# raguilar011095/planet_heightmap_generation

Hardware: AMD Instinct MI355X
Metric: Mcells·iter/s, terrain-post erosion stack (higher is better)
Workload: dtype f64

## Files before the change

### planet_heightmap_generation_amd/csrc/device.h

```cpp
#pragma once
#include <hip/hip_runtime.h>

#include <cstdint>
#include <cstdio>
#include <map>
#include <string>
#include <utility>
#include <vector>

#include "device_mem.h"
#include "host_util.h"

#include "erode_ops.h"
#include "flood_ops.h"
#include "wo_internal.h"

namespace wo {

#define WO_TRY try {
#define WO_CATCH(fn)                                                                                   \
    } catch (const ::wo::HipError& e) { ::wo::set_error(std::string(fn) + ": " + e.msg); return 2; }   \
      catch (const std::exception& e) { ::wo::set_error(std::string(fn) + ": " + e.what()); return 3; }

#define WO_LOCAL __attribute__((visibility("hidden")))
// ... 16 lines not shown
    const int64_t b = (n + WO_BLOCK - 1) / WO_BLOCK, per = 8 * (int64_t)xcd_tile(n);
    return (int)(((b + per - 1) / per) * per);
}

enum Family : int {
    FAM_COAST = 0, FAM_SMOOTH, FAM_SHARPEN, FAM_CREEP, FAM_WARP, FAM_NOISE, FAM_SYNTH, FAM_OCEAN,
    FAM_SORT_KEYS, FAM_SORT_RADIX, FAM_RANK, FAM_RECEIVERS, FAM_FLOW_SNAP, FAM_FLOW_FINAL,
    FAM_SOLVE_SETUP, FAM_SOLVE_ROUND, FAM_SOLVE_FINAL, FAM_THERMAL_EXCESS, FAM_THERMAL_APPLY,
    FAM_GLAC_INDEX, FAM_ICE_RECV, FAM_ICE_ROUND, FAM_CARVE_SETUP, FAM_CARVE_ROUND, FAM_MORAINE, FAM_GLAC_BLEND,
    FAM_SOLVE_PATCH, FAM_ELEV_COLLISION, FAM_ELEV_MAIN, FAM_PLATE_GRID, FAM_PLATE_PROJECT, FAM_SMOOTH_FIELD,
    FAM_FLOOD_EVAL, FAM_FLOOD_APPLY, FAM_FLOOD_MISC, FAM_CLIMATE, FAM_BASIN, FAM_BASIN_SORT, FAM_SOLVE_BASIN, FAM_FLOW_TILES, FAM_MISC, FAM_EVENT_PAIR, FAM_EVENT_PAIR_NOOP, FAM_EVENT_PAIR_NOOP2,
    FAM_MAP_LONLAT, FAM_MAP_FILL, FAM_MAP_SIDES, FAM_MAP_BIG_BOXES, FAM_MAP_RESOLVE, FAM_MAP_REGION_COLORS, FAM_MAP_PIXELS,
    FAM_MAP_RANGE, FAM_MAP_LAYER_COLORS,
    FAM_GLOBE_TABLES, FAM_GLOBE_REGION_COLORS, FAM_GLOBE_RANGE, FAM_GLOBE_MESH, FAM_GLOBE_LINE_COUNT, FAM_GLOBE_LINE_SCAN, FAM_GLOBE_LINE_WRITE,
    FAM_OVERLAY_BINS, FAM_OVERLAY_ARROWS,
    FAM_PICK, FAM_PICK_REDUCE, FAM_HIGHLIGHT, FAM_COUNT
};
extern const char* const kFamilyNames[FAM_COUNT];

}

struct wo_ctx {
    int device = 0;
    hipStream_t stream = nullptr;
    hipDeviceProp_t prop{};
};

struct wo_flood_gpu {
    wo::DeviceArena mem;
    int64_t version = -1; int32_t L = 0, cap = 0, nSeeds = 0;
    int32_t *off = nullptr, *adj = nullptr, *cell = nullptr, *seedIdx = nullptr, *seeds = nullptr; double* nz = nullptr;
    float* e = nullptr;
    wo::FlHead *A = nullptr, *P = nullptr, *F = nullptr;
    unsigned long long *Astk = nullptr, *Pstk = nullptr, *Fstk = nullptr;
    int32_t *fdEpoch = nullptr, *inDirty = nullptr; uint8_t* isPending = nullptr;
    int32_t* lists[5] = {nullptr, nullptr, nullptr, nullptr, nullptr};
    void* ctrl = nullptr; void* h_ctrl = nullptr;
    int32_t *jump = nullptr, *outPar = nullptr, *outRoot = nullptr; float* outSurf = nullptr;
    int32_t *h_par = nullptr, *h_root = nullptr; float* h_surf = nullptr;
};

namespace wo {
struct Options {
    bool layoutIndex = false;
    bool tileLds = false;
    bool floodDevice = false;
    bool floodTiming = false;
    bool stageTimingAll = false;
    int  relaxedSortEvery = 1;
    bool relaxedFull = false;
    bool basinScramble = false;
    long long carveBudgetMs = 200;
    int  carveBlocks = 0;
    bool oceanSplitSmooth = false;
    bool tempSplitDiffuse = false;
    bool globeDirectStores = false;
    bool overlayPrecheck = false;
    int  pickBlocks = 0;
    static Options from_env();
};
}

struct wo_planet {
    wo_ctx* ctx = nullptr;
    wo::Options opt;
    int32_t N = 0, E = 0, maxDeg = 0;
    wo::DeviceArena mem;
    wo::hvec<int32_t> h_off, h_adj;
    wo::hvec<float> h_xyz;
    wo::hvec<uint8_t> h_ocean;
    bool h_ocean_valid = false;
    float* h_pinned = nullptr;
    int32_t* h_count = nullptr;
    float* d_redoE = nullptr; int32_t* d_pendingEver = nullptr; int64_t redoCalls = 0;
    unsigned long long *h_word = nullptr, *d_word = nullptr; uint32_t wordSerial = 0;
    wo::FloodScratch flood;
    wo::FloodExchange floodX;
    void* floodLink = nullptr; void (*floodLinkFree)(void*) = nullptr;
    wo_flood_gpu fgpu;

    int32_t *d_off = nullptr, *d_adj = nullptr;
    float *d_dist = nullptr, *d_xyz = nullptr;
    float *d_e = nullptr, *d_e2 = nullptr, *d_hot = nullptr, *d_orig = nullptr;
    uint8_t *d_ocean = nullptr, *d_coast = nullptr;
    int64_t mirrorMaskVersion = -1;
    uint8_t* d_oceanKnown = nullptr; int32_t* d_maskDiff = nullptr; bool oceanKnownValid = false;
    bool hot_valid = false;
    float* d_savedE = nullptr; uint8_t* d_savedOcean = nullptr; bool saved = false;
    uint8_t* d_tables = nullptr;
    bool scratch = false;
    bool landIdentity = false;
    int64_t floodPrefixMirror = -1, floodPrefixStatic = -1;
    bool floodPrefixOk = false;
    int32_t *d_landIdx = nullptr, *d_land[2] = {nullptr, nullptr}, *d_rank = nullptr;
    int32_t* d_landInit = nullptr; int64_t oceanVersion = 0, landListsOcean = -1; bool landListsMirror = false; int32_t landListsL = -1;
    uint32_t* d_keys[2] = {nullptr, nullptr};
    float *d_cellDist = nullptr, *d_flow = nullptr;
    wo::SolveTask* d_task = nullptr; wo::SolveOut* d_out = nullptr;
    int32_t *d_haloSend = nullptr, *d_haloRecv = nullptr; float *d_haloBuf = nullptr, *h_haloBuf = nullptr; int32_t nHaloSend = 0, nHaloRecv = 0;
    int32_t* d_flowCnt = nullptr; wo::TargetRank* d_tr = nullptr; wo::EventList* d_ev = nullptr; float* d_me = nullptr;
    int32_t *d_carveSlot = nullptr, *d_carveDeps = nullptr, *d_carveDepCnt = nullptr, *d_carveDepPos = nullptr;
    uint32_t* d_rs[2] = {nullptr, nullptr}; int rsFlip[2] = {0, 0};
    wo::CarveRec* d_carveRecs = nullptr; wo::CarveExpect* d_carveExpect = nullptr; unsigned long long* d_carveG = nullptr;
    int32_t* d_carveSlotDone = nullptr; int64_t carveCap = 0;
    unsigned long long* d_accCnt = nullptr;
    int32_t *d_ftLr = nullptr, *d_ftParent = nullptr, *d_ftExtCnt = nullptr; uint32_t* d_ftInflow = nullptr; unsigned long long* d_ftRootAcc = nullptr;
// ... 137 lines not shown
```

### planet_heightmap_generation_amd/csrc/erode.hip

```cpp
#include <hip/hip_runtime.h>

#include <algorithm>
#include <chrono>
#include <cmath>

#include "../../include/worogen.h"
#include "device.h"
#include "flood.h"
#include "kernels_impl.h"
#include "mirror.h"
#include "stage_clock.h"

namespace wo {

__global__ __launch_bounds__(WO_BLOCK) void k_fill_i32(int32_t* a, int32_t v, int32_t n) { WO_GRID_STRIDE(i, n) a[i] = v; }

constexpr int WO_PATCH_TOTAL_SLOTS = 4096;

static void ensure_scratch(wo_planet* p) {
    if (p->scratch) return;
    const size_t N = (size_t)p->N;
    DeviceArena a;
    p->d_landIdx = a.dev<int32_t>(N); p->d_land[0] = a.dev<int32_t>(N); p->d_land[1] = a.dev<int32_t>(N);
    p->d_keys[0] = a.dev<uint32_t>(N); p->d_keys[1] = a.dev<uint32_t>(N);
// ... 27 lines not shown
        return 1;
    }
    int32_t* tot = p->d_patchTotals;
    int64_t launches = 0;
    constexpr int spinCap = WO_PATCH_SPIN_CAP, lateFrom = WO_PATCH_LATE_FROM, lateCap = WO_PATCH_LATE_SPIN_CAP;
    int64_t need = 0;
    for (int32_t tag = 1;; ) {
        const int32_t first = tag;
        const int burst = (tag == 1) ? std::max<int>(1, (int)std::min<int64_t>(p->lastPatchLaunches, WO_PATCH_TOTAL_SLOTS / 2)) : 3;
        for (int b = 0; b < burst; ++b, ++tag) {
            if (tag % WO_PATCH_TOTAL_SLOTS == 0) {
                if (b > 0) break;
                WO_HIP(hipMemsetAsync(tot, 0, (size_t)WO_PATCH_TOTAL_SLOTS * sizeof(int32_t), s));
            }
            if (tag == 1) basin_solve_launch(p, F, tag, tot + 1);
            else {
                if (tag == 2 && F.solveLean) launch(p, FAM_MISC, k_solve_blk_init, blocks_for(p->L, 4096), WO_BLOCK, F, p->L);
                launch(p, FAM_SOLVE_PATCH, k_solve_patch, np, WO_PATCH_THREADS, F, p->L, tag, p->d_patchPending, tot + (tag % WO_PATCH_TOTAL_SLOTS), K, m, dt,
                       (int32_t*)nullptr, (int32_t)(tag >= lateFrom ? lateCap : spinCap));
            }
            ++launches;
        }
        if (first == 1 && tag == 2) {
            if (read_count(p, tot + 1) == 0) need = 1;
        } else {
            WO_HIP(hipMemcpyAsync(p->h_patchTotals, tot, (size_t)WO_PATCH_TOTAL_SLOTS * sizeof(int32_t), hipMemcpyDeviceToHost, s));
            WO_HIP(hipStreamSynchronize(s));
            for (int32_t t = first; t < tag && !need; ++t) if (p->h_patchTotals[t % WO_PATCH_TOTAL_SLOTS] == 0) need = t;
        }
        if (need) break;
        if (launches > 4 * (int64_t)p->N + 1024) throw HipError{"patch solve does not converge"};
    }
    p->lastPatchLaunches = need;
    return need;
}

static void ensure_side_stream(wo_planet* p) {
    if (p->side) return;
    int prLeast = 0, prGreatest = 0;
    WO_HIP(hipDeviceGetStreamPriorityRange(&prLeast, &prGreatest));
    WO_HIP(hipStreamCreateWithPriority(&p->side, hipStreamNonBlocking, prGreatest));
    WO_HIP(hipEventCreateWithFlags(&p->evFork, hipEventDisableTiming)); WO_HIP(hipEventCreateWithFlags(&p->evJoin, hipEventDisableTiming));
}

struct RedoWithChecks {};

struct ErodeCall {
    wo_planet* p;
    int32_t hIters; double K, m, dt; int32_t tIters; double talus, kThermal; int32_t gIters; double gStrength; bool checkEveryPass;
    int32_t total, midIter; double gCarve, gConv, gDep, gFjord;
    int gridN, gridL = 0;
    StageClock clk; MirrorScope mir; FloodRun floodRun;
    int64_t sorts = 0, maxSolve = 0, patchLaunches = 0, basinPasses = 0, basinLeftoverPasses = 0, iceRounds = 0, carveRounds = 0, carveActive = 0, carveFlowLeft = 0;
    double floodHostMs = 0;
    ErodeCall(wo_planet* pl, int32_t h, double K_, double m_, double dt_, int32_t t, double talus_, double kT, int32_t g, double gs, bool check)
        : p(pl), hIters(h), K(K_), m(m_), dt(dt_), tIters(t), talus(talus_), kThermal(kT), gIters(std::max(g, 0)), gStrength(gs != gs ? 0 : gs),
          checkEveryPass(check), total(std::max(hIters, std::max(tIters, gIters))), midIter((int32_t)std::floor(total * 0.75 + 0.5)),
          gridN(xcd_grid(pl->N)), clk(pl), mir(pl) {
        const double gScale = gIters > 0 ? 1.0 / gIters : 0;
        gCarve = 0.02 * gScale; gConv = 0.01 * gScale; gDep = 0.005 * gScale; gFjord = 0.015 * gScale;
    }
    void stats(bool mirrored) const {
        p->erodeStats = {{"land_cells", (double)p->L}, {"mirror_layout", mirrored ? 1.0 : 0.0}, {"iterations", (double)total}, {"sorts", (double)sorts},
                         {"solve_launches_max_per_pass", (double)maxSolve}, {"solve_patch_launches_total", (double)patchLaunches},
                         {"solve_basin_passes", (double)basinPasses}, {"solve_basin_passes_with_leftovers", (double)basinLeftoverPasses},
                         {"flow_two_level", (p->d_ftLr && p->landIdentity && hIters > 0) ? 1.0 : 0.0}, {"ice_rounds_total", (double)iceRounds},
                         {"carve_rounds_total", (double)carveRounds}, {"carve_active_total", (double)carveActive}, {"carve_flow_launches_with_leftovers", (double)carveFlowLeft}, {"solve_check_every_pass", checkEveryPass ? 1.0 : 0.0}, {"calls_run_again_with_checks", (double)p->redoCalls}, {"flood_stage_ms", floodHostMs},
                         {"flood_device_pass1_ms", floodRun.deviceMs}, {"flood_device_rounds", (double)floodRun.rounds}, {"flood_device_epochs", (double)floodRun.epochs},
                         {"flood_device_evaluations", (double)floodRun.evals}, {"flood_equal_key_decisions", (double)floodRun.ties}, {"flood_pass1_on_host", (floodRun.usedDevice && !floodRun.fellBack) ? 0.0 : 1.0},
                         {"flood_host_calls", (double)floodRun.host.calls}, {"flood_host_serial_pass1", (double)floodRun.host.serialPass1}, {"flood_host_tie_groups", (double)floodRun.host.tieGroups}, {"flood_host_contested", (double)floodRun.host.contested},
                         {"flood_host_open_parents", (double)floodRun.host.openParents}, {"flood_host_unresolved", (double)floodRun.host.unresolved},
                         {"flood_host_path_redo", (double)floodRun.host.pathRedo}, {"flood_host_replays", (double)floodRun.host.replays}, {"flood_host_replayed_landmasses", (double)floodRun.host.replayedLandmasses}, {"flood_host_pass1_ms", floodRun.host.pass1Ms},
                         {"flood_host_pass23_ms", floodRun.host.pass23Ms},
                         {"relaxed_sort_every", (double)p->opt.relaxedSortEvery}, {"relaxed_full", p->opt.relaxedFull ? 1.0 : 0.0}, {"flood_exchange_calls", (double)p->floodX.calls}, {"flood_exchange_gathers", (double)p->floodX.gathers}, {"flood_exchange_whole_planet_floods", (double)p->floodX.globalFloods}, {"flood_exchange_received", (double)p->floodX.received}};
    }
};
template <class Cell>
static int32_t compact_land(int64_t n, const uint8_t* ocean, Cell cell, int32_t* out) {
    std::vector<int64_t> cnt(host_threads() + 2, 0);
    parallel_ranges(n, [&](int64_t b, int64_t e, int t) { int64_t c = 0; for (int64_t i = b; i < e; ++i) c += ocean[cell(i)] ? 0 : 1; cnt[t + 1] = c; });
    for (size_t t = 1; t < cnt.size(); ++t) cnt[t] += cnt[t - 1];
    parallel_ranges(n, [&](int64_t b, int64_t e, int t) { int64_t o = cnt[t]; for (int64_t i = b; i < e; ++i) if (!ocean[cell(i)]) out[o++] = (int32_t)i; });
    return (int32_t)cnt.back();
}
static void erode_without_land(ErodeCall& c) {
    wo_planet* p = c.p;
    if (p->floodX.on) {
        hipStream_t s = p->ctx->stream;
        const int calls = (c.hIters > 0 ? 1 : 0) + (c.midIter < c.total ? 1 : 0);
        WO_HIP(hipMemcpyAsync(p->h_pinned, c.mir.on ? p->mirror.o_e : p->d_e, (size_t)p->N * sizeof(float), hipMemcpyDeviceToHost, s));
        WO_HIP(hipStreamSynchronize(s));
        ensure_flood_static(p);
        for (int k = 0; k < calls; ++k) flood_exchange(p, 0.5, nullptr);
    }
    c.mir.finish();
    c.clk.end(); c.clk.finish();
}
static bool erode_setup(ErodeCall& c) {
    wo_planet* p = c.p; hipStream_t s = p->ctx->stream;
    const int32_t N = p->N;
    c.clk.begin("setup");
    refresh_host_ocean(p);
    c.mir.enter(p->h_ocean.data());
    p->landIdentity = c.mir.on && p->mirror.h_mask.size() == (size_t)N;
    coast_flags(p);
    int32_t* hl = reinterpret_cast<int32_t*>(p->h_pinned);
    const uint8_t* oc = p->h_ocean.data();
    const bool listsKept = p->d_landInit && p->landListsOcean == p->oceanVersion && p->landListsMirror == c.mir.on && p->landListsL >= 0;
    const int32_t L = listsKept ? p->landListsL : compact_land(N, oc, [](int64_t r) { return r; }, hl);
    p->L = L;
    if (L == 0) { erode_without_land(c); return false; }
    if (listsKept) {
        WO_HIP(hipMemcpyAsync(p->d_land[0], p->d_landInit, (size_t)L * sizeof(int32_t), hipMemcpyDeviceToDevice, s));
    } else if (c.mir.on) {
        WO_HIP(hipMemcpyAsync(p->d_listA, hl, (size_t)L * sizeof(int32_t), hipMemcpyHostToDevice, s));
        mirror_map_i32(p, p->d_listA, p->d_land[0], L);
        WO_HIP(hipStreamSynchronize(s));
        const int32_t* perm = p->mirror.h_perm.data();
        compact_land(N, oc, [perm](int64_t i) { return perm[i]; }, hl);
        WO_HIP(hipMemcpyAsync(p->d_landIdx, hl, (size_t)L * sizeof(int32_t), hipMemcpyHostToDevice, s));
    } else {
        WO_HIP(hipMemcpyAsync(p->d_landIdx, hl, (size_t)L * sizeof(int32_t), hipMemcpyHostToDevice, s));
        WO_HIP(hipMemcpyAsync(p->d_land[0], p->d_landIdx, (size_t)L * sizeof(int32_t), hipMemcpyDeviceToDevice, s));
    }
    if (!listsKept) {
        if (!p->d_landInit) p->d_landInit = p->mem.dev<int32_t>((size_t)N);
        WO_HIP(hipMemcpyAsync(p->d_landInit, p->d_land[0], (size_t)L * sizeof(int32_t), hipMemcpyDeviceToDevice, s));
        p->landListsOcean = p->oceanVersion; p->landListsMirror = c.mir.on; p->landListsL = L;
    }
    WO_HIP(hipStreamSynchronize(s));
    p->landCur = 0;
    launch(p, FAM_MISC, k_init_rank, c.gridN, WO_BLOCK, p->d_rank, N);
    rank_from_land(p);
    if (c.hIters > 0) {
        ensure_flood_static(p);
        if (p->patchVersion != p->flood.staticVersion || p->patchMirror != c.mir.on) {
            p->patchMirror = c.mir.on;
            if (c.mir.on) WO_HIP(hipMemcpyAsync(p->d_patchOrder, p->d_landIdx, (size_t)L * sizeof(int32_t), hipMemcpyDeviceToDevice, s));
            else WO_HIP(hipMemcpyAsync(p->d_patchOrder, p->flood.landCell.data(), (size_t)L * sizeof(int32_t), hipMemcpyHostToDevice, s));
            launch(p, FAM_MISC, k_fill_i32, c.gridN, WO_BLOCK, p->d_slotOf, -1, N);
            launch(p, FAM_MISC, k_slot_scatter, blocks_for(L, 4096), WO_BLOCK, (const int32_t*)p->d_patchOrder, p->d_slotOf, L);
            WO_HIP(hipStreamSynchronize(s));
            p->patchVersion = p->flood.staticVersion;
            p->lastPatchLaunches = 1;
            p->numPatches = (L + WO_PATCH - 1) / WO_PATCH;
        }
    } else p->patchVersion = -1;
    c.gridL = xcd_grid(L);
    if (c.hIters > 0 || c.tIters > 0) {
        WO_HIP(hipMemcpyAsync(p->d_e2, p->d_e, (size_t)N * sizeof(float), hipMemcpyDeviceToDevice, s));
        launch(p, FAM_MISC, k_erode_ocean_init, blocks_for(N, 4096), WO_BLOCK, p->fields());
    }
    c.clk.end();
    return true;
}
static void leftovers_so_far(ErodeCall& c) {
    wo_planet* p = c.p;
    if (c.checkEveryPass || !p->d_pendingEver || read_count(p, p->d_pendingEver) == 0) return;
    if (p->opt.floodTiming) {
        int32_t h[8] = {0};
        WO_HIP(hipMemcpy(h, p->d_pendingEver, sizeof(h), hipMemcpyDeviceToHost));
        std::fprintf(stderr, "[erode] call runs again with checks: %d basin-solve tasks were left pending\n", h[0]);
    }
    throw RedoWithChecks{};
}
static void erode_flood(ErodeCall& c, double carveStrength) {
    wo_planet* p = c.p;
    leftovers_so_far(c);
    c.clk.begin("priority_flood");
    const auto t0 = std::chrono::steady_clock::now();
    const bool landOnly = c.mir.on && p->landIdentity && !p->floodX.on && !p->opt.floodDevice && p->h_ocean_valid && p->flood.staticValid &&
                          p->flood.staticN == p->N && p->flood.L > 0 && flood_land_is_mirror_prefix(p);
    if (landOnly) flood_stage_land(p, carveStrength, c.floodRun);
    else { c.mir.suspend(); flood_stage(p, carveStrength, c.floodRun); c.mir.resume(); }
    c.floodHostMs += std::chrono::duration<double, std::milli>(std::chrono::steady_clock::now() - t0).count();
    c.clk.end();
}
static void erode_sort(ErodeCall& c) { c.clk.begin("sort"); sort_land_by_elevation(c.p); ++c.sorts; c.clk.end(); }
static void ice_flow(ErodeCall& c, const Fields& F) {
    launch(c.p, FAM_ICE_RECV, k_ice_receivers, c.gridN, WO_BLOCK, F);
    launch(c.p, FAM_ICE_ROUND, k_ice_climb, c.gridL, WO_BLOCK, F, F.blocker); ++c.iceRounds;
}
static void glacial_step_relaxed(ErodeCall& c) {
    wo_planet* p = c.p;
    c.clk.begin("glacial");
    const Fields F = p->fields();
    ice_flow(c, F);
    launch(p, FAM_CARVE_ROUND, k_carve_jacobi, c.gridL, WO_BLOCK, F, (const float*)p->d_e, p->d_e2, c.gCarve, c.gConv, c.gStrength);
    swap_elev(p);
    launch(p, FAM_MORAINE, k_moraine_fjord, c.gridN, WO_BLOCK, p->fields(), c.gDep, c.gFjord);
    c.clk.end();
}
static void ensure_carve_capacity(wo_planet* p, int32_t active) {
    if ((int64_t)active <= p->carveCap) return;
    DeviceArena& a = p->mem;
    a.release(p->d_carveDeps); a.release(p->d_carveDepCnt); a.release(p->d_carveDepPos); a.release(p->d_carveRecs); a.release(p->d_carveSlotDone); a.release(p->d_carveExpect);
    p->carveCap = 0;
    const size_t cap = (size_t)active + active / 4 + 1024;
    p->d_carveDeps = a.dev<int32_t>(cap * WO_CARVE_DEPS);
    p->d_carveDepCnt = a.dev<int32_t>(cap); p->d_carveDepPos = a.dev<int32_t>(cap);
    p->d_carveRecs = a.dev<CarveRec>(cap); p->d_carveSlotDone = a.dev<int32_t>(cap); p->d_carveExpect = a.dev<CarveExpect>(cap);
    p->carveCap = (int64_t)cap;
}
static int carve_granule_blocks() {
    static int blocks = 0;
    if (!blocks) {
        int perCu = 0, dev = 0; hipDeviceProp_t prop;
        WO_HIP(hipOccupancyMaxActiveBlocksPerMultiprocessor(&perCu, k_carve_granules, WO_BLOCK, 0));
        WO_HIP(hipGetDevice(&dev)); WO_HIP(hipGetDeviceProperties(&prop, dev));
        blocks = std::max(1, std::min(perCu, 8) - 1) * prop.multiProcessorCount;
    }
    return blocks;
}
static int64_t carve_launches(ErodeCall& c, const Fields& F, int32_t active) {
    wo_planet* p = c.p;
    const int32_t* const count = p->d_counters + 3; int32_t* const done = p->d_counters + 4;
    launch(p, FAM_CARVE_SETUP, k_carve_records, blocks_for(active), WO_BLOCK, F, (const int32_t*)p->d_listB, count, p->d_carveRecs, p->d_carveSlotDone, c.gCarve, c.gConv, c.gStrength,
           (int32_t)0, (int32_t)1);
    WO_HIP(hipMemsetAsync(done, 0, sizeof(int32_t), p->ctx->stream));
    const int grid = blocks_for(active);
    const int blocksNow = p->opt.carveBlocks > 0 ? std::max(1, std::min(carve_granule_blocks(), p->opt.carveBlocks)) : carve_granule_blocks();
    const long long flowBudget = p->opt.carveBudgetMs * 100000ll;
    if (!p->d_carveG) p->d_carveG = p->mem.dev<unsigned long long>((size_t)p->N);
    launch(p, FAM_CARVE_SETUP, k_carve_expect, grid, WO_BLOCK, F, (const CarveRec*)p->d_carveRecs, count, p->d_carveExpect);
    launch(p, FAM_CARVE_SETUP, k_carve_pack, blocks_for(p->N, 4096), WO_BLOCK, (const float*)F.e, p->d_carveG, p->N);
    launch(p, FAM_CARVE_ROUND, k_carve_granules, std::min(grid, blocksNow), WO_BLOCK, F, (const CarveRec*)p->d_carveRecs, (const CarveExpect*)p->d_carveExpect, p->d_carveG,
           p->d_carveSlotDone, count, done, flowBudget);
    launch(p, FAM_CARVE_SETUP, k_carve_unpack, blocks_for(p->N, 4096), WO_BLOCK, (const unsigned long long*)p->d_carveG, F.e, p->N);
    int64_t k = 2;
    if (read_count(p, done) >= active) return k - 1;
    ++c.carveFlowLeft;
    launch(p, FAM_CARVE_SETUP, k_carve_deps, grid, WO_BLOCK, F, (const int32_t*)p->d_listB, count, p->d_carveSlot);
    launch(p, FAM_CARVE_SETUP, k_carve_records, grid, WO_BLOCK, F, (const int32_t*)p->d_listB, count, p->d_carveRecs, p->d_carveSlotDone, c.gCarve, c.gConv, c.gStrength, (int32_t)1, (int32_t)0);
    constexpr int burst = 32;
    for (;;) {
        for (int b = 0; b < burst; ++b, ++k)
            launch(p, FAM_CARVE_ROUND, k_carve_round_static, grid, WO_BLOCK, F, (const CarveRec*)p->d_carveRecs, p->d_carveSlotDone, count, (int32_t)k, c.gCarve, c.gConv, c.gStrength, done);
        if (read_count(p, done) >= active) return k - 1;
        if (k > 4 * (int64_t)p->N + 1024) throw HipError{"carve rounds do not converge"};
    }
}
static void glacial_step_exact(ErodeCall& c) {
    wo_planet* p = c.p;
    c.clk.begin("glacial");
    Fields F = p->fields();
    ice_flow(c, F);
    launch(p, FAM_CARVE_SETUP, k_carve_setup_cells, c.gridN, WO_BLOCK, F);
    select_active_by_rank(p, F.arank, p->d_listB, p->d_counters + 3);
    const int32_t active = read_count(p, p->d_counters + 3);
    c.carveActive += active; ensure_carve_capacity(p, active);
    F.carveDeps = p->d_carveDeps; F.carveDepCnt = p->d_carveDepCnt; F.carveDepPos = p->d_carveDepPos;
    if (active > 0) c.carveRounds += carve_launches(c, F, active);
    launch(p, FAM_MORAINE, k_moraine_fjord, c.gridN, WO_BLOCK, F, c.gDep, c.gFjord);
    c.clk.end();
}
static FlowTiles flow_tiles_buffers(wo_planet* p) {
    const size_t N = (size_t)p->N;
    if (!p->d_ftLr) {
        DeviceArena& a = p->mem;
        if (!p->d_ftParent) p->d_ftParent = a.dev<int32_t>(N);
        if (!p->d_ftExtCnt) p->d_ftExtCnt = a.dev<int32_t>(N);
        if (!p->d_ftInflow) p->d_ftInflow = a.dev<uint32_t>(N);
        if (!p->d_ftRootAcc) p->d_ftRootAcc = a.dev<unsigned long long>(N);
        p->d_ftLr = a.dev<int32_t>(N);
        WO_HIP(hipMemsetAsync(p->d_ftInflow, 0, N * 4, p->ctx->stream)); WO_HIP(hipMemsetAsync(p->d_ftExtCnt, 0, N * 4, p->ctx->stream));
    }
    FlowTiles FT{};
    FT.lr = p->d_ftLr; FT.parent = p->d_ftParent; FT.rootAcc = p->d_ftRootAcc; FT.inflow = p->d_ftInflow; FT.extCnt = p->d_ftExtCnt;
    return FT;
}
static int flow_tile_count(int32_t L) { return (int)(((int64_t)L + FT_CELLS - 1) / FT_CELLS); }
static void erode_receivers(ErodeCall& c, const Fields& F, const FlowTiles& FT, int32_t* donorCnt, bool basin, bool slotIdentity, bool tilesBeforeFork) {
    wo_planet* p = c.p; hipStream_t s = p->ctx->stream;
    Fields Fr = F; if (basin) Fr.basinJ = p->d_basinJ;
    c.clk.begin("receivers");
    launch(p, FAM_RECEIVERS, k_receivers_flow_init, c.gridL, WO_BLOCK, Fr, donorCnt);
    c.clk.end();
    if (!basin) return;
    ensure_side_stream(p);
    if (tilesBeforeFork) {
        launch(p, FAM_FLOW_TILES, k_flow_tiles<false>, flow_tile_count(p->L), FT_THREADS, F, FT);
        launch(p, FAM_FLOW_TILES, k_flow_root_links, blocks_for(p->L, 4096), WO_BLOCK, F, FT);
    }
    WO_HIP(hipEventRecord(p->evFork, s));
    WO_HIP(hipStreamWaitEvent(p->side, p->evFork, 0));
    p->onSide = true;
    try { basin_layout(p, slotIdentity); } catch (...) { p->onSide = false; throw; }
    p->onSide = false;
    WO_HIP(hipEventRecord(p->evJoin, p->side));
}
static void erode_flow(ErodeCall& c, const Fields& F, const FlowTiles& FT, int32_t* donorCnt, bool flowTiles, bool tilesBeforeFork, bool clearOut) {
    wo_planet* p = c.p;
    c.clk.begin("flow");
    if (flowTiles) {
        const int tiles = flow_tile_count(p->L);
        if (!tilesBeforeFork) {
            launch(p, FAM_FLOW_TILES, k_flow_tiles<false>, tiles, FT_THREADS, F, FT);
            launch(p, FAM_FLOW_TILES, k_flow_root_links, blocks_for(p->L, 4096), WO_BLOCK, F, FT);
        }
        launch(p, FAM_FLOW_TILES, k_flow_root_climb, blocks_for(p->L, 4096), WO_BLOCK, F, FT);
        launch(p, FAM_FLOW_TILES, k_flow_tiles<true>, tiles, FT_THREADS, F, FT);
    } else
        launch(p, FAM_FLOW_SNAP, k_flow_climb, c.gridL, WO_BLOCK, F, (const int32_t*)p->d_flowCnt, (int32_t)0x7fffffff);
    Fields Ff = F;
    if (p->opt.relaxedFull) Ff.ev = nullptr;
// ... 41 lines not shown
    erode_flow(c, F, FT, donorCnt, flowTiles, tilesBeforeFork, basin && c.checkEveryPass);
    c.clk.begin("solve");
    if (basin) erode_solve_basin(c, F, iter); else erode_solve_affine(c, F);
    swap_elev(p);
    c.clk.end();
}
static void thermal_step(ErodeCall& c, bool afterSolve) {
    wo_planet* p = c.p;
    c.clk.begin("thermal");
    const Fields F = p->fields();
    if (!afterSolve) launch(p, FAM_THERMAL_EXCESS, k_masked_elev, c.gridL, WO_BLOCK, F);
    launch(p, FAM_THERMAL_EXCESS, k_thermal_excess, c.gridL, WO_BLOCK, F, c.talus);
    if (p->maxDeg <= 12) launch(p, FAM_THERMAL_APPLY, k_thermal_apply_reg<12>, c.gridL, WO_BLOCK, F, p->d_e2, c.talus, c.kThermal);
    else if (p->maxDeg <= 16) launch(p, FAM_THERMAL_APPLY, k_thermal_apply_reg<16>, c.gridL, WO_BLOCK, F, p->d_e2, c.talus, c.kThermal);
    else launch_shmem(p, FAM_THERMAL_APPLY, k_thermal_apply, c.gridL, WO_BLOCK, (size_t)p->maxDeg * WO_BLOCK * 12, F, p->d_e2, c.talus, c.kThermal, (int32_t)p->maxDeg);
    swap_elev(p);
    c.clk.end();
}

static void erode_composite(wo_planet* p, int32_t hIters, double K, double m, double dt, int32_t tIters, double talus,
                            double kThermal, int32_t gIters, double gStrength, bool checkEveryPass = true) {
    ErodeCall c(p, hIters, K, m, dt, tIters, talus, kThermal, gIters, gStrength, checkEveryPass);
    release_stage_brackets(p);
    p->stageTiming.clear(); p->erodeStats.clear();
    p->floodX.calls = 0; p->floodX.gathers = 0; p->floodX.globalFloods = 0; p->floodX.received = 0;
    if (c.total <= 0) return;
    ensure_scratch(p);
    hipStream_t s = p->ctx->stream;
    if (hIters > 0) WO_HIP(hipMemsetAsync(p->d_flowCnt, 0, (size_t)p->N * sizeof(int32_t), s));
    if (hIters > 0 && p->d_ftInflow) { WO_HIP(hipMemsetAsync(p->d_ftInflow, 0, (size_t)p->N * 4, s)); WO_HIP(hipMemsetAsync(p->d_ftExtCnt, 0, (size_t)p->N * 4, s)); }
    if (!erode_setup(c)) return;
    if (hIters > 0) erode_flood(c, 0.5);

    const bool glacial = c.gIters > 0 && c.gStrength > 0;
    if (glacial) launch(p, FAM_GLAC_INDEX, k_glac_index, c.gridN, WO_BLOCK, p->fields(), c.gStrength);
    const bool relaxedFull = p->opt.relaxedFull;
    bool midDone = false, sortAfterFlood = false;
    for (int32_t iter = 0; iter < c.total; ++iter) {
        c.clk.on = true;
        if (!midDone && iter >= c.midIter) { midDone = true; erode_flood(c, 0.85); sortAfterFlood = true; }
        c.clk.on = p->opt.stageTimingAll || p->profiling || c.total <= 16 || iter % 8 == 0;
        const bool gNow = iter < c.gIters && glacial, hNow = iter < hIters;
        const bool sortNow = relaxedFull ? (iter == 0 || sortAfterFlood) : (p->opt.relaxedSortEvery <= 1 || iter % p->opt.relaxedSortEvery == 0);
        if ((gNow || hNow) && sortNow) { sortAfterFlood = false; erode_sort(c); }
        if (gNow) { if (relaxedFull) glacial_step_relaxed(c); else glacial_step_exact(c); }
        if (hNow) {
            if (gNow && sortNow) erode_sort(c);
            hydraulic_step(c, iter);
        }
        if (iter < tIters) thermal_step(c, hNow);
    }
    c.clk.on = true;
    leftovers_so_far(c);
    if (glacial) {
        c.clk.begin("glacial_blend");
        launch(p, FAM_GLAC_BLEND, k_glacial_blend, c.gridN, WO_BLOCK, p->fields(), (const float*)p->d_e, p->d_e2);
        swap_elev(p);
        c.clk.end();
    }
    const bool mirrored = c.mir.on;
    if (mirrored) { c.clk.begin("setup"); c.mir.finish(); c.clk.end(); }
    c.clk.finish();
    c.stats(mirrored);
}

static void erode_composite_checked(wo_planet* p, int32_t hIters, double K, double m, double dt, int32_t tIters, double talus,
                                    double kThermal, int32_t gIters, double gStrength) {
    if (hIters <= 0 || p->floodX.on) { erode_composite(p, hIters, K, m, dt, tIters, talus, kThermal, gIters, gStrength, true); return; }
    hipStream_t s = p->ctx->stream;
    if (!p->d_redoE) p->d_redoE = p->mem.dev<float>((size_t)p->N);
    if (!p->d_pendingEver) p->d_pendingEver = p->mem.dev<int32_t>(16);
    WO_HIP(hipMemcpyAsync(p->d_redoE, p->d_e, (size_t)p->N * sizeof(float), hipMemcpyDeviceToDevice, s));
    WO_HIP(hipMemsetAsync(p->d_pendingEver, 0, 16 * sizeof(int32_t), s));
    try {
        erode_composite(p, hIters, K, m, dt, tIters, talus, kThermal, gIters, gStrength, false);
    } catch (const RedoWithChecks&) {
        WO_HIP(hipStreamSynchronize(s));
        if (p->side) WO_HIP(hipStreamSynchronize(p->side));
        WO_HIP(hipMemcpyAsync(p->d_e, p->d_redoE, (size_t)p->N * sizeof(float), hipMemcpyDeviceToDevice, s));
        ++p->redoCalls;
        erode_composite(p, hIters, K, m, dt, tIters, talus, kThermal, gIters, gStrength, true);
    }
}

}

using namespace wo;

extern "C" {

int wo_erode_composite_resident(wo_planet* p, int32_t hIters, double K, double m, double dt, int32_t tIters, double talusSlope,
                                double kThermal, int32_t gIters, double glacialStrength) {
    if (!check_planet(p, "wo_erode_composite_resident")) return 1;
    WO_TRY
    erode_composite_checked(p, hIters, K, m, dt, tIters, talusSlope, kThermal, gIters, glacialStrength);
    return 0;
    WO_CATCH("wo_erode_composite_resident")
}

struct ErodeArgs { int32_t h; double K, m, dt; int32_t t; double talus, kT; int32_t g; double gs; };
int wo_erode_composite(wo_planet* p, float* e, const uint8_t* oc, int32_t hIters, double K, double m, double dt, int32_t tIters,
                       double talusSlope, double kThermal, int32_t gIters, double glacialStrength) {
    ErodeArgs a{hIters, K, m, dt, tIters, talusSlope, kThermal, gIters, glacialStrength};
    return with_host_field(p, "wo_erode_composite", e, oc, true,
                           [](wo_planet* q, void* v) { auto* x = (ErodeArgs*)v; erode_composite_checked(q, x->h, x->K, x->m, x->dt, x->t, x->talus, x->kT, x->g, x->gs); }, &a);
}
// ... 3 lines not shown
```

### planet_heightmap_generation_amd/csrc/kernels_impl.h

```cpp
#pragma once
#include <hip/hip_runtime.h>

#include "common_kernels.h"
#include "device.h"

namespace wo {

#define WO_XCD_LAND(i, r)                                                                                            \
    for (int32_t xi_ = (int32_t)(blockIdx.x >> 3), xt_ = F.xcdTileL,                                                 \
                 i = (int32_t)((((xi_ / xt_) * 8 + (int32_t)(blockIdx.x & 7u)) * xt_ + (xi_ % xt_)) * (int32_t)blockDim.x + (int32_t)threadIdx.x), \
                 once_ = 1;                                                                                          \
         once_ && i < F.L; once_ = 0)                                                                                \
        for (int32_t r = F.landIdx ? F.landIdx[i] : i, once2_ = 1; once2_; once2_ = 0)


__global__ __launch_bounds__(WO_BLOCK) void k_init_rank(int32_t* rank, int32_t N) { WO_GRID_STRIDE(r, N) rank[r] = -1; }

__global__ __launch_bounds__(WO_BLOCK) void k_erode_ocean_init(Fields F) {
    WO_GRID_STRIDE(r, F.N) {
        if (!F.ocean[r]) continue;
        if (F.target) F.target[r] = -1;
        TargetRank z; z.target = -1; z.rank = -1; F.tr[r] = z;
        if (F.accA) F.accA[r] = 0;
        F.jumpA[r] = -1; F.flow[r] = 0.0f; F.totalExcess[r] = 0.0; F.me[r] = INFINITY;
// ... 585 lines not shown

__global__ __launch_bounds__(WO_BLOCK) void k_carve_setup_cells(Fields F) {
    WO_XCD_CELLS(r, F.N) carve_setup_cell(F, r);
}
__global__ __launch_bounds__(WO_BLOCK) void k_carve_deps(Fields F, const int32_t* list, const int32_t* count, int32_t* carveSlot) {
    const int32_t n = *count;
    WO_GRID_STRIDE(i, n) { const int32_t r = list[i]; carveSlot[r] = i; carve_deps_cell(F, r, i); }
}
__global__ __launch_bounds__(WO_BLOCK) void k_carve_records(Fields F, const int32_t* list, const int32_t* count, CarveRec* recs, int32_t* slotDone, double gCarve, double gConv, double gStrength,
                                                             int32_t withDeps, int32_t resetDone) {
    const int32_t n = *count;
    WO_GRID_STRIDE(i, n) { carve_record_cell(F, list[i], i, recs, gCarve, gConv, gStrength, withDeps); if (resetDone) slotDone[i] = WO_NOT_DONE; }
}
__global__ __launch_bounds__(WO_BLOCK) void k_carve_round_static(Fields F, const CarveRec* __restrict__ recs, int32_t* slotDone, const int32_t* __restrict__ count, int32_t round,
                                                                  double gCarve, double gConv, double gStrength, int32_t* done) {
    const int32_t n = *count;
    const int32_t i = blockIdx.x * blockDim.x + threadIdx.x;
    bool ran = false;
    if (i < n && slotDone[i] == WO_NOT_DONE) {
        const CarveRec R = recs[i];
        ran = carve_task_rec(F, R, i, round, gCarve, gConv, gStrength);
        if (ran) slotDone[i] = round;
    }
    const unsigned long long m = __ballot(ran);
    if (m && (threadIdx.x & 63) == 0) atomicAdd(done, __popcll(m));
}
__device__ inline unsigned long long granule_pack(float v, int32_t tag) { return ((unsigned long long)(uint32_t)tag << 32) | (unsigned long long)__float_as_uint(v); }
__device__ inline float granule_value(unsigned long long g) { return __uint_as_float((uint32_t)g); }
__device__ inline int32_t granule_tag(unsigned long long g) { return (int32_t)(g >> 32); }
__device__ inline unsigned long long ld_agent(const unsigned long long* p) { return __hip_atomic_load(p, __ATOMIC_RELAXED, __HIP_MEMORY_SCOPE_AGENT); }
__device__ inline void st_agent(unsigned long long* p, unsigned long long v) { __hip_atomic_store(p, v, __ATOMIC_RELAXED, __HIP_MEMORY_SCOPE_AGENT); }
__device__ inline int32_t carve_expected_tag(const Fields& F, int32_t x, int32_t myRank) {
    int32_t m = -1;
    { const int32_t a = F.arank[x]; if (a < myRank) m = a; }
    for (int32_t j = F.off[x]; j < F.off[x + 1]; ++j) { const int32_t a = F.arank[F.adj[j]]; if (a < myRank && a > m) m = a; }
    return m + 1;
}
__global__ __launch_bounds__(WO_BLOCK) void k_carve_expect(Fields F, const CarveRec* __restrict__ recs, const int32_t* __restrict__ count, CarveExpect* ex) {
    const int32_t n = *count;
    WO_GRID_STRIDE(i, n) {
        const int32_t r = recs[i].r, deg = recs[i].deg, myRank = F.arank[r];
        CarveExpect X;
        X.myTag = myRank + 1; X.pad_[0] = X.pad_[1] = 0;
        for (int k = 0; k <= WO_EAGER_ROW; ++k) X.tag[k] = -1;
        if (deg <= WO_EAGER_ROW) {
            const int32_t b = F.off[r];
            for (int k = 0; k < deg; ++k) { const int32_t x = F.adj[b + k]; if (!F.ocean[x]) X.tag[k] = carve_expected_tag(F, x, myRank); }
            X.tag[WO_EAGER_ROW] = carve_expected_tag(F, r, myRank);
        }
        ex[i] = X;
    }
}
__global__ __launch_bounds__(WO_BLOCK) void k_carve_pack(const float* __restrict__ e, unsigned long long* __restrict__ G, int32_t n) { WO_GRID_STRIDE(i, n) G[i] = granule_pack(e[i], 0); }
__global__ __launch_bounds__(WO_BLOCK) void k_carve_unpack(const unsigned long long* __restrict__ G, float* __restrict__ e, int32_t n) { WO_GRID_STRIDE(i, n) e[i] = granule_value(G[i]); }
__device__ inline bool carve_granule_turn_long_row(const Fields& F, unsigned long long* G, int32_t r, double deepening, double bonus, int32_t up) {
    const int32_t myRank = F.arank[r], myTag = myRank + 1;
    if (granule_tag(ld_agent(&G[r])) != carve_expected_tag(F, r, myRank)) return false;
    for (int32_t j = F.off[r]; j < F.off[r + 1]; ++j) {
        const int32_t nb = F.adj[j];
        if (!F.ocean[nb] && granule_tag(ld_agent(&G[nb])) != carve_expected_tag(F, nb, myRank)) return false;
    }
    float er = (float)((double)granule_value(ld_agent(&G[r])) - deepening);
    for (int32_t j = F.off[r]; j < F.off[r + 1]; ++j) {
        const int32_t nb = F.adj[j];
        if (F.ocean[nb]) continue;
        const double d = nd_or_eps(F.dist[j]);
        const float en = granule_value(ld_agent(&G[nb]));
        const double slope = fabs((double)er - (double)en) / d;
        double f = 1 - slope;
        if (!(f > 0)) f = (f != f) ? f : 0;
        st_agent(&G[nb], granule_pack((float)((double)en - deepening * 0.4 * f), myTag));
    }
    if (up >= 2) er = (float)((double)er - bonus);
    st_agent(&G[r], granule_pack(er, myTag));
    return true;
}
__global__ __launch_bounds__(WO_BLOCK, 4) void k_carve_granules(Fields F, const CarveRec* __restrict__ recs, const CarveExpect* __restrict__ expect, unsigned long long* G,
                                                              int32_t* slotDone, const int32_t* __restrict__ count, int32_t* done, long long budget) {
    const int32_t n = *count;
    const int32_t stride = (int32_t)(gridDim.x * blockDim.x);
    int32_t i = (int32_t)(blockIdx.x * blockDim.x + threadIdx.x);
    const long long t0 = wall_clock64();
    int32_t finished = 0;
    bool active = i < n;
    int32_t r = 0, deg = 0, up = 0, nbs[WO_EAGER_ROW]; float dist[WO_EAGER_ROW]; double deepening = 0, bonus = 0;
    CarveExpect X;
    float vals[WO_EAGER_ROW + 1];
    uint32_t pend = 0;
    auto fetch = [&]() {
        const CarveRec& R = recs[i];
        r = R.r; deg = R.deg; up = R.up; deepening = R.deepening; bonus = R.bonus;
#pragma unroll
        for (int k = 0; k < WO_EAGER_ROW; ++k) { nbs[k] = R.nbs[k]; dist[k] = R.dist[k]; }
        X = expect[i];
        pend = 0;
#pragma unroll
        for (int k = 0; k <= WO_EAGER_ROW; ++k) if (X.tag[k] >= 0) pend |= 1u << k;
    };
    if (active) fetch();
    for (;;) {
        if (active) {
            bool ran = false;
            if (deg > WO_EAGER_ROW) ran = carve_granule_turn_long_row(F, G, r, deepening, bonus, up);
            else {
                unsigned long long g[WO_EAGER_ROW + 1];
#pragma unroll
                for (int k = 0; k <= WO_EAGER_ROW; ++k) g[k] = ((pend >> k) & 1u) ? ld_agent(&G[k < WO_EAGER_ROW ? nbs[k] : r]) : 0ull;
// ... 111 lines not shown
```

### planet_heightmap_generation_amd/csrc/planet.hip

```cpp
#include <hip/hip_runtime.h>

#include <algorithm>
#include <atomic>
#include <chrono>
#include <cstring>

#include "../../include/worogen.h"
#include "common_kernels.h"
#include "device.h"

wo::Fields wo_planet::fields() const {
    wo::Fields F{};
    F.N = N; F.xcdTile = wo::xcd_tile(N); F.tileLds = opt.tileLds ? 1 : 0; F.off = d_off; F.adj = d_adj; F.dist = d_dist; F.xyz = d_xyz; F.ocean = d_ocean; F.coast = d_coast;
    F.e = d_e; F.e2 = d_e2; F.L = L; F.land = d_land[landCur]; F.landIdx = landIdentity ? nullptr : d_landIdx; F.xcdTileL = wo::xcd_tile(L > 0 ? L : 1); F.rank = d_rank; F.target = nullptr; F.tr = d_tr; F.ev = d_ev; F.me = d_me; F.carveSlot = d_carveSlot; F.carveDeps = nullptr; F.carveDepCnt = d_carveDepCnt; F.carveDepPos = d_carveDepPos; F.cellDist = d_cellDist;
    F.flow = d_flow; F.accA = nullptr; F.accB = nullptr; F.accCnt = d_accCnt; F.jumpA = d_jump; F.jumpB = nullptr;
    F.task = d_task; F.out = d_out; F.slotOf = (patchVersion >= 0) ? d_slotOf : nullptr; F.blk = d_patchBlk; F.doneAt = d_doneAt;
    F.totalExcess = d_totalExcess; F.glac = d_glac; F.iceTarget = d_iceTarget; F.iceFlow = d_iceFlow; F.iceUp = d_iceUp; F.arank = d_arank; F.blocker = d_nj;
    return F;
}

namespace wo {

__global__ __launch_bounds__(WO_BLOCK) void k_ocean_from_elev(const float* e, uint8_t* ocean, int32_t N) {
    WO_GRID_STRIDE(r, N) ocean[r] = (e[r] <= 0.0f) ? 1 : 0;
// ... 29 lines not shown
    }
    p->h_ocean_valid = true;
    if (!p->d_maskDiff) p->d_maskDiff = p->mem.dev<int32_t>(1);
    if (!p->d_oceanKnown) p->d_oceanKnown = p->mem.dev<uint8_t>(p->N);
    WO_HIP(hipMemcpyAsync(p->d_oceanKnown, p->d_ocean, (size_t)p->N, hipMemcpyDeviceToDevice, s));
    p->oceanKnownValid = true;
}

int32_t read_count(wo_planet* p, const int32_t* d_ptr) {
    hipStream_t s = p->ctx->stream;
    if (!p->h_word) {
        p->h_word = p->mem.try_pinned<unsigned long long>(8, hipHostMallocMapped);
        if (!p->h_word || hipHostGetDevicePointer((void**)&p->d_word, p->h_word, 0) != hipSuccess) { p->mem.release(p->h_word); p->d_word = nullptr; (void)hipGetLastError(); }
        else *p->h_word = 0;
    }
    if (p->h_word) {
        const uint32_t serial = ++p->wordSerial;
        hipLaunchKernelGGL(k_publish_count, dim3(1), dim3(1), 0, s, d_ptr, p->d_word, serial);
        const auto t0 = std::chrono::steady_clock::now();
        for (uint64_t spins = 0;; ++spins) {
            const unsigned long long w = __atomic_load_n(p->h_word, __ATOMIC_ACQUIRE);
            if ((uint32_t)(w >> 32) == serial) return (int32_t)(uint32_t)w;
            if ((spins & 0xfff) == 0xfff && std::chrono::steady_clock::now() - t0 > std::chrono::seconds(2)) break;
            __builtin_ia32_pause();
        }
        WO_HIP(hipStreamSynchronize(s));
        const unsigned long long w = __atomic_load_n(p->h_word, __ATOMIC_ACQUIRE);
        if ((uint32_t)(w >> 32) == serial) return (int32_t)(uint32_t)w;
    }
    WO_HIP(hipMemcpyAsync(p->h_count, d_ptr, sizeof(int32_t), hipMemcpyDeviceToHost, s));
    WO_HIP(hipStreamSynchronize(s));
    return p->h_count[0];
}

}

using namespace wo;

Options Options::from_env() {
    auto str = [](const char* n) { const char* v = std::getenv(n); return std::string(v ? v : ""); };
    auto on = [](const char* n) { const char* v = std::getenv(n); return v && std::atoi(v) != 0; };
    auto set = [](const char* n) { return std::getenv(n) != nullptr; };
    Options o;
    o.layoutIndex = str("WO_LAYOUT") == "index";
    o.tileLds = on("WO_TILE_LDS");
    o.floodDevice = str("WO_FLOOD") == "device";
    o.floodTiming = set("WO_FLOOD_TIMING");
    o.stageTimingAll = str("WO_STAGE_TIMING") == "all";
    if (set("WO_RELAXED_SORT_EVERY")) o.relaxedSortEvery = std::max(1, std::atoi(std::getenv("WO_RELAXED_SORT_EVERY")));
    o.relaxedFull = str("WO_RELAXED") == "full";
    o.basinScramble = test_hook_int("basin_scramble", 0) != 0;
    o.carveBudgetMs = test_hook_int("carve_budget_ms", 200);
    o.carveBlocks = (int)std::max<long long>(0, test_hook_int("carve_blocks", 0));
    o.oceanSplitSmooth = test_hook_int("ocean_split_smooth", 0) != 0;
    o.tempSplitDiffuse = test_hook_int("temp_split_diffuse", 0) != 0;
    o.globeDirectStores = test_hook_int("globe_direct_stores", 0) != 0;
    o.overlayPrecheck = test_hook_int("overlay_precheck", 0) != 0;
    o.pickBlocks = (int)std::max<long long>(0, std::min<long long>(test_hook_int("pick_blocks", 0), 1 << 16));
    return o;
}

bool wo::check_planet(wo_planet* p, const char* fn) {
    if (!p) { set_error(std::string(fn) + ": null planet handle"); return false; }
    p->opt = Options::from_env();
    hipError_t e = hipSetDevice(p->ctx->device);
    if (e != hipSuccess) { set_error(std::string(fn) + ": hipSetDevice failed: " + hipGetErrorString(e)); return false; }
    return true;
}

extern "C" {

int wo_device_count(void) {
    int n = 0;
    if (hipGetDeviceCount(&n) != hipSuccess) return 0;
    return n;
}

wo_ctx* wo_ctx_create(int32_t device) {
    try {
        int n = 0;
        if (hipGetDeviceCount(&n) != hipSuccess || n <= 0) {
            set_error("wo_ctx_create: no usable HIP device (libworogen has no CPU fallback)");
            return nullptr;
        }
        if (device < 0 || device >= n) { set_error("wo_ctx_create: device index out of range"); return nullptr; }
        auto* c = new wo_ctx();
        c->device = device;
        WO_HIP(hipSetDevice(device));
        WO_HIP(hipGetDeviceProperties(&c->prop, device));
        WO_HIP(hipStreamCreateWithFlags(&c->stream, hipStreamNonBlocking));
        return c;
    } catch (const HipError& e) { set_error(std::string("wo_ctx_create: ") + e.msg); return nullptr; }
}

void wo_ctx_destroy(wo_ctx* c) {
    if (!c) return;
    (void)hipSetDevice(c->device);
    if (c->stream) (void)hipStreamDestroy(c->stream);
    delete c;
}

wo_planet* wo_planet_create(wo_ctx* ctx, int32_t numRegions, const int32_t* adjOffset, const int32_t* adjList,
                            const float* r_xyz, const float* neighborDist) {
    if (!ctx || numRegions < 1 || !adjOffset || !adjList || !r_xyz) { set_error("wo_planet_create: bad arguments"); return nullptr; }
    wo_planet* p = nullptr;
    try {
// ... 279 lines not shown
```

Measured before the change: 6400.

## Defer glacial carve count readback using device-side bound and leftover tracking

Removes the per-iteration host readback of the active carve count and the completion check by launching carve kernels with a fixed upper bound (capacity or L). A new device-side setup kernel resets the done counter and accumulates stats, and it flags overflow or unfinished tasks into the pending counters. At the end of the call these counters are checked, and the whole call is re-run with checks if anything was left open. The pack and unpack kernels are also limited to land cells when the layout is identity. The cost is over-launched grids sized to the bound and possible full re-runs when carving does not finish.

```diff
diff --git a/planet_heightmap_generation_amd/csrc/device.h b/planet_heightmap_generation_amd/csrc/device.h
--- a/planet_heightmap_generation_amd/csrc/device.h
+++ b/planet_heightmap_generation_amd/csrc/device.h
@@ -92,6 +92,7 @@
     bool basinScramble = false;
     long long carveBudgetMs = 200;
     int  carveBlocks = 0;
+    int  carveBound = 0;
     bool oceanSplitSmooth = false;
     bool tempSplitDiffuse = false;
     bool globeDirectStores = false;
diff --git a/planet_heightmap_generation_amd/csrc/erode.hip b/planet_heightmap_generation_amd/csrc/erode.hip
--- a/planet_heightmap_generation_amd/csrc/erode.hip
+++ b/planet_heightmap_generation_amd/csrc/erode.hip
@@ -103,6 +103,7 @@
     int gridN, gridL = 0;
     StageClock clk; MirrorScope mir; FloodRun floodRun;
     int64_t sorts = 0, maxSolve = 0, patchLaunches = 0, basinPasses = 0, basinLeftoverPasses = 0, iceRounds = 0, carveRounds = 0, carveActive = 0, carveFlowLeft = 0;
+    int32_t carveBound = 0;
     double floodHostMs = 0;
     ErodeCall(wo_planet* pl, int32_t h, double K_, double m_, double dt_, int32_t t, double talus_, double kT, int32_t g, double gs, bool check)
         : p(pl), hIters(h), K(K_), m(m_), dt(dt_), tIters(t), talus(talus_), kThermal(kT), gIters(std::max(g, 0)), gStrength(gs != gs ? 0 : gs),
@@ -207,11 +208,13 @@
 }
 static void leftovers_so_far(ErodeCall& c) {
     wo_planet* p = c.p;
-    if (c.checkEveryPass || !p->d_pendingEver || read_count(p, p->d_pendingEver) == 0) return;
+    if (c.checkEveryPass || !p->d_pendingEver) return;
+    const bool glacial = c.gIters > 0 && c.gStrength > 0 && !p->opt.relaxedFull;
+    if (read_count(p, p->d_pendingEver) == 0 && (!glacial || read_count(p, p->d_pendingEver + 1) == 0)) return;
     if (p->opt.floodTiming) {
         int32_t h[8] = {0};
         WO_HIP(hipMemcpy(h, p->d_pendingEver, sizeof(h), hipMemcpyDeviceToHost));
-        std::fprintf(stderr, "[erode] call runs again with checks: %d basin-solve tasks were left pending\n", h[0]);
+        std::fprintf(stderr, "[erode] call runs again with checks: %d basin-solve tasks were left pending, %d carve tasks left open\n", h[0], h[1]);
     }
     throw RedoWithChecks{};
 }
@@ -263,23 +266,25 @@
     }
     return blocks;
 }
-static int64_t carve_launches(ErodeCall& c, const Fields& F, int32_t active) {
+static int64_t carve_launches(ErodeCall& c, const Fields& F, int32_t active, bool deferred) {
     wo_planet* p = c.p;
     const int32_t* const count = p->d_counters + 3; int32_t* const done = p->d_counters + 4;
+    launch(p, FAM_CARVE_SETUP, k_carve_begin, 1, 1, p->d_counters + 3, done, active, deferred ? p->d_pendingEver : (int32_t*)nullptr);
     launch(p, FAM_CARVE_SETUP, k_carve_records, blocks_for(active), WO_BLOCK, F, (const int32_t*)p->d_listB, count, p->d_carveRecs, p->d_carveSlotDone, c.gCarve, c.gConv, c.gStrength,
            (int32_t)0, (int32_t)1);
-    WO_HIP(hipMemsetAsync(done, 0, sizeof(int32_t), p->ctx->stream));
     const int grid = blocks_for(active);
+    const int32_t cells = p->landIdentity ? p->L : p->N;
     const int blocksNow = p->opt.carveBlocks > 0 ? std::max(1, std::min(carve_granule_blocks(), p->opt.carveBlocks)) : carve_granule_blocks();
     const long long flowBudget = p->opt.carveBudgetMs * 100000ll;
     if (!p->d_carveG) p->d_carveG = p->mem.dev<unsigned long long>((size_t)p->N);
     launch(p, FAM_CARVE_SETUP, k_carve_expect, grid, WO_BLOCK, F, (const CarveRec*)p->d_carveRecs, count, p->d_carveExpect);
-    launch(p, FAM_CARVE_SETUP, k_carve_pack, blocks_for(p->N, 4096), WO_BLOCK, (const float*)F.e, p->d_carveG, p->N);
+    launch(p, FAM_CARVE_SETUP, k_carve_pack, blocks_for(cells, 4096), WO_BLOCK, (const float*)F.e, p->d_carveG, cells);
     launch(p, FAM_CARVE_ROUND, k_carve_granules, std::min(grid, blocksNow), WO_BLOCK, F, (const CarveRec*)p->d_carveRecs, (const CarveExpect*)p->d_carveExpect, p->d_carveG,
            p->d_carveSlotDone, count, done, flowBudget);
-    launch(p, FAM_CARVE_SETUP, k_carve_unpack, blocks_for(p->N, 4096), WO_BLOCK, (const unsigned long long*)p->d_carveG, F.e, p->N);
+    launch(p, FAM_CARVE_SETUP, k_carve_unpack, blocks_for(cells, 4096), WO_BLOCK, (const unsigned long long*)p->d_carveG, F.e, cells, count, (const int32_t*)done,
+           deferred ? p->d_pendingEver + 1 : (int32_t*)nullptr);
     int64_t k = 2;
-    if (read_count(p, done) >= active) return k - 1;
+    if (deferred || read_count(p, done) >= active) return k - 1;
     ++c.carveFlowLeft;
     launch(p, FAM_CARVE_SETUP, k_carve_deps, grid, WO_BLOCK, F, (const int32_t*)p->d_listB, count, p->d_carveSlot);
     launch(p, FAM_CARVE_SETUP, k_carve_records, grid, WO_BLOCK, F, (const int32_t*)p->d_listB, count, p->d_carveRecs, p->d_carveSlotDone, c.gCarve, c.gConv, c.gStrength, (int32_t)1, (int32_t)0);
@@ -298,10 +303,20 @@
     ice_flow(c, F);
     launch(p, FAM_CARVE_SETUP, k_carve_setup_cells, c.gridN, WO_BLOCK, F);
     select_active_by_rank(p, F.arank, p->d_listB, p->d_counters + 3);
-    const int32_t active = read_count(p, p->d_counters + 3);
-    c.carveActive += active; ensure_carve_capacity(p, active);
+    const bool deferred = !c.checkEveryPass;
+    int32_t active;
+    if (deferred && c.carveBound > 0) active = c.carveBound;
+    else {
+        active = read_count(p, p->d_counters + 3);
+        ensure_carve_capacity(p, active);
+        if (deferred && active > 0) {
+            active = c.carveBound = (int32_t)std::min<int64_t>(p->carveCap, p->L);
+            if (p->opt.carveBound > 0) active = c.carveBound = std::min(active, p->opt.carveBound);
+        }
+        else c.carveActive += active;
+    }
     F.carveDeps = p->d_carveDeps; F.carveDepCnt = p->d_carveDepCnt; F.carveDepPos = p->d_carveDepPos;
-    if (active > 0) c.carveRounds += carve_launches(c, F, active);
+    if (active > 0) { const int64_t k = carve_launches(c, F, active, deferred); if (!deferred) c.carveRounds += k; }
     launch(p, FAM_MORAINE, k_moraine_fjord, c.gridN, WO_BLOCK, F, c.gDep, c.gFjord);
     c.clk.end();
 }
@@ -449,6 +464,12 @@
     }
     c.clk.on = true;
     leftovers_so_far(c);
+    if (glacial && !checkEveryPass && !relaxedFull) {
+        int32_t h[8] = {0};
+        WO_HIP(hipMemcpyAsync(h, p->d_pendingEver, sizeof(h), hipMemcpyDeviceToHost, s));
+        WO_HIP(hipStreamSynchronize(s));
+        c.carveRounds = h[2]; c.carveActive = (int64_t)(((uint64_t)(uint32_t)h[5] << 32) | (uint32_t)h[4]);
+    }
     if (glacial) {
         c.clk.begin("glacial_blend");
         launch(p, FAM_GLAC_BLEND, k_glacial_blend, c.gridN, WO_BLOCK, p->fields(), (const float*)p->d_e, p->d_e2);
diff --git a/planet_heightmap_generation_amd/csrc/kernels_impl.h b/planet_heightmap_generation_amd/csrc/kernels_impl.h
--- a/planet_heightmap_generation_amd/csrc/kernels_impl.h
+++ b/planet_heightmap_generation_amd/csrc/kernels_impl.h
@@ -661,7 +661,20 @@
     }
 }
 __global__ __launch_bounds__(WO_BLOCK) void k_carve_pack(const float* __restrict__ e, unsigned long long* __restrict__ G, int32_t n) { WO_GRID_STRIDE(i, n) G[i] = granule_pack(e[i], 0); }
-__global__ __launch_bounds__(WO_BLOCK) void k_carve_unpack(const unsigned long long* __restrict__ G, float* __restrict__ e, int32_t n) { WO_GRID_STRIDE(i, n) e[i] = granule_value(G[i]); }
+__global__ __launch_bounds__(WO_BLOCK) void k_carve_unpack(const unsigned long long* __restrict__ G, float* __restrict__ e, int32_t n, const int32_t* __restrict__ count,
+                                                            const int32_t* __restrict__ done, int32_t* leftOpen) {
+    WO_GRID_STRIDE(i, n) e[i] = granule_value(G[i]);
+    if (leftOpen && blockIdx.x == 0 && threadIdx.x == 0) { const int32_t open = *count - *done; if (open > 0) *leftOpen += open; }
+}
+__global__ void k_carve_begin(int32_t* count, int32_t* done, int32_t cap, int32_t* pend) {
+    if (blockIdx.x != 0 || threadIdx.x != 0) return;
+    *done = 0;
+    if (!pend) return;
+    const int32_t n = *count;
+    *reinterpret_cast<unsigned long long*>(pend + 4) += (unsigned long long)n;
+    if (n > 0) pend[2] += 1;
+    if (n > cap) { pend[1] += n; *count = 0; }
+}
 __device__ inline bool carve_granule_turn_long_row(const Fields& F, unsigned long long* G, int32_t r, double deepening, double bonus, int32_t up) {
     const int32_t myRank = F.arank[r], myTag = myRank + 1;
     if (granule_tag(ld_agent(&G[r])) != carve_expected_tag(F, r, myRank)) return false;
diff --git a/planet_heightmap_generation_amd/csrc/planet.hip b/planet_heightmap_generation_amd/csrc/planet.hip
--- a/planet_heightmap_generation_amd/csrc/planet.hip
+++ b/planet_heightmap_generation_amd/csrc/planet.hip
@@ -105,6 +105,7 @@
     o.basinScramble = test_hook_int("basin_scramble", 0) != 0;
     o.carveBudgetMs = test_hook_int("carve_budget_ms", 200);
     o.carveBlocks = (int)std::max<long long>(0, test_hook_int("carve_blocks", 0));
+    o.carveBound = (int)std::max<long long>(0, std::min<long long>(test_hook_int("carve_bound", 0), 0x7fffffff));
     o.oceanSplitSmooth = test_hook_int("ocean_split_smooth", 0) != 0;
     o.tempSplitDiffuse = test_hook_int("temp_split_diffuse", 0) != 0;
     o.globeDirectStores = test_hook_int("globe_direct_stores", 0) != 0;
```

After: 6390 (median of 2 runs). No clear change (-0.2%).
